# cswaney/NetworkHawkesProcesses.jl

Measured on AMD Instinct MI355X. Metric: log-likelihood evals/sec (N=1024, M=1e6), higher is better.
Workload: dtype f64; 1 GPU; continuous exponential standard Hawkes, N=1024, M=1000000, dt_max=1, windowed_k8 (S-metric, SURVEY 8d); pairs_per_eval=7999107, independent_streams=1

## Files before the change

networkhawkesprocesses.jl_amd/csrc/cont_slices.hip:

```cpp
#include <algorithm>
#include <vector>

#include "nhp_internal.h"
#include "nhp_math.h"
#include "nhp_rng.h"

struct nhp_slices {
    const uint32_t *row;
    const int32_t *item0;
    const uint32_t *lo;
    const uint16_t *hi;
    int32_t nsh;
    uint32_t dmask;
    int32_t dbits;
};

#define NHP_SL_SHARDS 64

#ifdef NHP_STAMP
__device__ unsigned long long g_sl_stamps[8 * 4096];
__device__ unsigned long long g_sl_wave_end[16 * 4096];
#define NHP_SL_STAMP(i) do { if (threadIdx.x == 0 && blockIdx.x < 4096) g_sl_stamps[8 * blockIdx.x + (i)] = __builtin_amdgcn_s_memrealtime(); } while (0)
#define NHP_SL_STAMP_WAVE() do { if ((threadIdx.x & 63) == 0 && blockIdx.x < 4096) g_sl_wave_end[16 * blockIdx.x + (threadIdx.x >> 6)] = __builtin_amdgcn_s_memrealtime(); } while (0)
extern "C" int nhp_debug_stamps_slices(unsigned long long *out, int n)
// ... 147 lines not shown
    for (int k = it.kbeg + threadIdx.x; k < it.kend; k += 256) {
        const nhp_child ch = a.child_w[k];
        const uint32_t slot = (uint32_t)(k - it.kbeg);
        for (int j = ch.idx - 1; j >= ch.first; --j) {
            const nhp_event e = a.ev[j];
            const uint32_t pos = atomicAdd(&cursor[e.node], 1u);
            const int rk = rankof[(size_t)blockIdx.x * N + e.node];
            double q = __builtin_rint((ch.t - e.t) * scale);
            q = q < 1.0 ? 1.0 : (q > qmax ? qmax : q);
            const uint64_t qi = (uint64_t)q;
            const size_t o = ((size_t)row[rk >> 6] + pos) * 64 + (size_t)(rk & 63);
            lo[o] = (uint32_t)qi;
            hi[o] = (uint16_t)((slot << ps.psh) | (uint32_t)(qi >> 32));
        }
    }
    for (int rk = threadIdx.x; rk < ps.spi * 64; rk += 256) {
        const int p = ps.perm[(size_t)blockIdx.x * ps.spi * 64 + rk];
        const uint32_t n = p == 0xFFFF ? 0u : cnt[(size_t)blockIdx.x * N + p];
        const uint32_t r0 = row[rk >> 6], R = row[(rk >> 6) + 1] - r0;
        for (uint32_t i = n; i < R; ++i) {
            const size_t o = ((size_t)r0 + i) * 64 + (size_t)(rk & 63);
            lo[o] = 0;
            hi[o] = (uint16_t)((uint32_t)ps.max_item << ps.psh);
        }
    }
}

__global__ __launch_bounds__(256) void k_ps_sort(int N, nhp_pslices ps, const uint32_t *__restrict__ cnt, uint32_t *__restrict__ lo,
                                                 uint16_t *__restrict__ hi)
{
    const uint32_t *row = ps.row + (size_t)blockIdx.x * ps.spi;
    for (int rk = threadIdx.x; rk < ps.spi * 64; rk += 256) {
        const int p = ps.perm[(size_t)blockIdx.x * ps.spi * 64 + rk];
        if (p == 0xFFFF) continue;
        const int n = (int)cnt[(size_t)blockIdx.x * N + p];
        const size_t o0 = (size_t)row[rk >> 6] * 64 + (size_t)(rk & 63);
        for (int i = 1; i < n; ++i) {
            const uint32_t l = lo[o0 + (size_t)i * 64], h = hi[o0 + (size_t)i * 64];
            const uint64_t key = ((uint64_t)h << 32) | l;
            int j = i - 1;
            while (j >= 0) {
                const uint32_t lj = lo[o0 + (size_t)j * 64], hj = hi[o0 + (size_t)j * 64];
                if ((((uint64_t)hj << 32) | lj) <= key) break;
                lo[o0 + (size_t)(j + 1) * 64] = lj;
                hi[o0 + (size_t)(j + 1) * 64] = (uint16_t)hj;
                --j;
            }
            lo[o0 + (size_t)(j + 1) * 64] = l;
            hi[o0 + (size_t)(j + 1) * 64] = (uint16_t)h;
        }
    }
}

template <int BLOCK, int C, bool FLAT, bool GRAD>
__global__ __launch_bounds__(BLOCK) void k_windowed_slices(nhp_cont_args a, nhp_slices sl, nhp_pslices ps, int mask_integral,
                                                            double *__restrict__ partials, unsigned int *__restrict__ counter,
                                                            double *__restrict__ out, int defer)
{
    constexpr int NW = BLOCK / 64;
    extern __shared__ __align__(16) unsigned char smem[];
    double *red = reinterpret_cast<double *>(smem);
    double2 *col = reinterpret_cast<double2 *>(smem + 320);
    double *etab = reinterpret_cast<double *>(col + a.N + 1);
    double *ginv = etab + 64;
    const int tid = threadIdx.x, lane = tid & 63;
    const double tab_v = nhp_exp2_64[lane];

    const nhp_item it = a.items[blockIdx.x];
    const int c = it.node, N = a.N;
    const int w = __builtin_amdgcn_readfirstlane(tid >> 6);
    const int nchild = it.kend - it.kbeg;
    const int s0 = sl.item0[blockIdx.x], ns = sl.item0[blockIdx.x + 1] - s0;
    NHP_SL_STAMP(0);

    struct chunk { uint32_t lo[C], hi[C]; };
    auto request = [&](chunk &q, const uint32_t *plo, const uint16_t *phi, const uint32_t row0, const int r) {
        const size_t o = ((size_t)row0 + (size_t)r) * 64;
        const uint32_t *pl = plo + o;
        const uint16_t *ph = phi + o;
#pragma unroll
        for (int u = 0; u < C; ++u) {
            q.lo[u] = pl[u * 64 + lane];
            q.hi[u] = ph[u * 64 + lane];
        }
    };
    constexpr int UN = BLOCK >= 512 ? 2 : 4;
    const double unit = __builtin_ldexp(a.dt_max, -sl.dbits);
    int j = w;
    uint32_t row0 = 0;
    int K = 0;
    chunk qa, qb;
    double integ = 0.0;
    for (int p0 = 0; p0 < N; p0 += UN * BLOCK) {
        double w_[UN], th_[UN], a_[UN], cnt_[UN];
#pragma unroll
        for (int u = 0; u < UN; ++u) {
            const int p = p0 + u * BLOCK + tid;
            const size_t k = (size_t)(p < N ? p : 0) + (size_t)c * N;
            w_[u] = a.W[k];
            th_[u] = a.p1[k];
            a_[u] = a.A ? a.A[k] : 1.0;
            cnt_[u] = it.first ? a.cnt[p < N ? p : 0] : 0.0;
        }
        if (p0 == 0) {
            if (j < ns) { row0 = sl.row[s0 + j]; K = (int)(sl.row[s0 + j + 1] - row0); }
            asm volatile("" ::: "memory");
            request(qa, sl.lo, sl.hi, row0, 0);
            asm volatile("" ::: "memory");
        }
#pragma unroll
        for (int u = 0; u < UN; ++u) {
            const int p = p0 + u * BLOCK + tid;
            if (p < N) {
                double wv = w_[u], wint = wv;
                if (a.A) {
                    wv = a_[u] * wv;
                    if (mask_integral) wint = wv;
                }
                col[p] = make_double2(-((th_[u] * unit) * 92.33248261689366), wv * th_[u]);
                integ += cnt_[u] * wint;
            }
        }
    }
    if (tid < 64) etab[tid] = tab_v;
    if (tid == 0) col[N] = make_double2(0.0, 0.0);
    if (GRAD && tid == 0) ginv[ps.max_item] = 0.0;
    if (out && it.first) integ += sl_baseline_integral_col(a, c);
    __syncthreads();
    NHP_SL_STAMP(1);

    const double lam0 = FLAT ? a.lambda0[c] : 0.0;
    const uint32_t dmask = sl.dmask;
    const int nsh = sl.nsh;
    auto delay = [&](const uint32_t lo, const uint32_t h, const uint32_t mask) {
        uint32_t hw;
        asm("v_bfi_b32 %0, %1, %2, %3" : "=v"(hw) : "s"(mask), "v"(h), "v"(0x43300000u));
        return __hiloint2double((int)hw, (int)lo) - 4503599627370496.0;
    };
    auto term = [&](const uint32_t lo, const uint32_t h) {
        const double v = delay(lo, h, dmask);
        const double2 cw = col[h >> nsh];
        return cw.y * nhp_exp_neg_tab_scaled(cw.x * v, etab);
    };
    auto sum = [&](const chunk &q, const int r, const int K, double s) {
        if (r + C <= K) {
            double t[C];
#pragma unroll
            for (int u = 0; u < C; ++u) t[u] = term(q.lo[u], q.hi[u]);
#pragma unroll
            for (int u = 0; u < C; ++u) s += t[u];
        } else {
#pragma unroll
            for (int u = 0; u < C; ++u)
                if (r + u < K) s += term(q.lo[u], q.hi[u]);
        }
        return s;
    };
    double prod = 1.0, gsum = 0.0;
    int pexp = 0;
    int rnd = 0;
    while (j < ns) {
        const int jn = nhp_slice_of(++rnd, w, NW);
        uint32_t row0n = 0;
        int Kn = 0;
        if (jn < ns) { row0n = sl.row[s0 + jn]; Kn = (int)(sl.row[s0 + jn + 1] - row0n); }
        double s = 0.0;
        if (K <= 0) request(qa, sl.lo, sl.hi, row0n, 0);
        for (int r0 = 0; r0 < K; r0 += 2 * C) {
            request(qb, sl.lo, sl.hi, row0, r0 + C);
            asm volatile("" ::: "memory");
            s = sum(qa, r0, K, s);
            const bool more = r0 + 2 * C < K;
            request(qa, sl.lo, sl.hi, more ? row0 : row0n, more ? r0 + 2 * C : 0);
            asm volatile("" ::: "memory");
            s = sum(qb, r0 + C, K, s);
        }
        const int kk = 64 * j + lane;
        if (kk < nchild) {
            const double tk = FLAT ? 0.0 : a.child_w[it.kbeg + kk].t;
            const double lam = (FLAT ? lam0 : sl_baseline(a, c, tk)) + s;
// ... 39 lines not shown
        __syncthreads();
        auto gterm = [&](const uint32_t lo, const uint32_t h, const double xs, double &accH, double &acc1) {
            const double v = delay(lo, h, pmask);
            const double g = ginv[h >> psh];
            const double t = xs * v;
            const double ge = g * nhp_exp_neg_tab_scaled(t, etab);
            accH += ge;
            acc1 = __builtin_fma(ge, __builtin_fma(t, 1.0830424696249145e-02, 1.0), acc1);
        };
        auto gsum_chunk = [&](const chunk &q, const int r, const int K, const double xs, double &accH, double &acc1) {
            if (r + C <= K) {
#pragma unroll
                for (int u = 0; u < C; ++u) gterm(q.lo[u], q.hi[u], xs, accH, acc1);
            } else {
#pragma unroll
                for (int u = 0; u < C; ++u)
                    if (r + u < K) gterm(q.lo[u], q.hi[u], xs, accH, acc1);
            }
        };
        while (jp < ps.spi) {
            const int jn = jp + NW;
            uint32_t row0n = 0;
            int Kn = 0;
            if (jn < ps.spi) { row0n = prow[jn]; Kn = (int)(prow[jn + 1] - row0n); }
            const lanep nxt = lane_params(jn);
            const double xs = -((cur.th * punit) * 92.33248261689366);
            double accH = 0.0, acc1 = 0.0;
            if (Kp <= 0) request(qa, ps.lo, ps.hi, row0n, 0);
            for (int r0 = 0; r0 < Kp; r0 += 2 * C) {
                request(qb, ps.lo, ps.hi, prow0, r0 + C);
                asm volatile("" ::: "memory");
                gsum_chunk(qa, r0, Kp, xs, accH, acc1);
                const bool more = r0 + 2 * C < Kp;
                request(qa, ps.lo, ps.hi, more ? prow0 : row0n, more ? r0 + 2 * C : 0);
                asm volatile("" ::: "memory");
                gsum_chunk(qb, r0 + C, Kp, xs, accH, acc1);
            }
            if (cur.p != 0xFFFF) {
                const size_t k = (size_t)cur.p + (size_t)c * N;
                const double gW = cur.av * (cur.th * accH);
                const double gT = (cur.av * cur.wv) * acc1;
                if (ps.direct) {
                    const double mk = (a.A && mask_integral) ? cur.av : 1.0;
                    ps.grad[L.W + k] = gW - cur.cn * mk;
                    ps.grad[L.p1 + k] = gT;
                } else {
                    if (gW != 0.0) atomicAdd(&ps.grad[L.W + k], gW);
                    if (gT != 0.0) atomicAdd(&ps.grad[L.p1 + k], gT);
                }
            }
            jp = jn; prow0 = row0n; Kp = Kn; cur = nxt;
        }
    }
    double acc = nhp_log(prod) + (double)pexp * 6.93147180559945286e-01;
    if (prod == 0.0) acc = -__builtin_inf();
    double blk = acc, blk_int = integ;
    nhp_block_sum2_n<NW>(blk, blk_int, red);
    if (GRAD && FLAT) {
        const double gs = nhp_block_sum_n<NW>(gsum, red);
        if (tid == 0) {
            if (ps.direct) ps.grad[c] = gs - a.duration;
            else if (gs != 0.0) atomicAdd(&ps.grad[c], gs);
        }
        __syncthreads();
    }
    NHP_SL_STAMP(3);
    if (!out || defer) {
        if (tid == 0) {
            partials[2 * (size_t)blockIdx.x] = blk;
            partials[2 * (size_t)blockIdx.x + 1] = blk_int;
        }
        NHP_SL_STAMP(4);
        return;
    }
    int *flag = reinterpret_cast<int *>(red + 32);
    if (tid == 0) {
        __hip_atomic_store(&partials[2 * (size_t)blockIdx.x], blk, __ATOMIC_RELAXED, __HIP_MEMORY_SCOPE_AGENT);
        __hip_atomic_store(&partials[2 * (size_t)blockIdx.x + 1], blk_int, __ATOMIC_RELAXED, __HIP_MEMORY_SCOPE_AGENT);
        asm volatile("s_waitcnt vmcnt(0)" ::: "memory");
        const unsigned int nb = gridDim.x, sh = blockIdx.x % NHP_SL_SHARDS;
        const unsigned int pop = (nb - sh + NHP_SL_SHARDS - 1) / NHP_SL_SHARDS;
        const unsigned int used = nb < NHP_SL_SHARDS ? nb : NHP_SL_SHARDS;
        int last = 0;
        if (__hip_atomic_fetch_add(&counter[32 * (1 + sh)], 1u, __ATOMIC_RELAXED, __HIP_MEMORY_SCOPE_AGENT) == pop - 1)
            last = __hip_atomic_fetch_add(&counter[0], 1u, __ATOMIC_RELAXED, __HIP_MEMORY_SCOPE_AGENT) == used - 1;
        *flag = last;
    }
    __syncthreads();
    NHP_SL_STAMP(4);
    if (!*flag) return;
    double sl_ = 0.0, si = 0.0;
    for (unsigned int i = tid; i < gridDim.x; i += BLOCK) {
        sl_ += __hip_atomic_load(&partials[2 * (size_t)i], __ATOMIC_RELAXED, __HIP_MEMORY_SCOPE_AGENT);
        si += __hip_atomic_load(&partials[2 * (size_t)i + 1], __ATOMIC_RELAXED, __HIP_MEMORY_SCOPE_AGENT);
    }
    nhp_block_sum2_n<NW>(sl_, si, red);
    if (tid == 0) *out = (0.0 - si) + sl_;
    for (int i = tid; i <= NHP_SL_SHARDS; i += BLOCK)
        __hip_atomic_store(&counter[32 * i], 0u, __ATOMIC_RELAXED, __HIP_MEMORY_SCOPE_AGENT);
}

#define NHP_SETS_MAX 4
struct nhp_sets {
    const double *p1[NHP_SETS_MAX], *W[NHP_SETS_MAX], *A[NHP_SETS_MAX], *lambda0[NHP_SETS_MAX];
    double *out[NHP_SETS_MAX];
};

__device__ __forceinline__ double sl_flat_integral(const double lam0, const double duration)
{
#pragma clang fp contract(off)
    return threadIdx.x == 0 ? lam0 * duration : 0.0;
}

__device__ __forceinline__ double sl_log_of(const double prod, const int pexp)
{
#pragma clang fp contract(off)
    const double e = (double)pexp * 6.93147180559945286e-01;
    return e + nhp_log(prod);
}

template <int BLOCK, int C, int S, bool DEFER = false>
__global__ __launch_bounds__(BLOCK) void k_slices_batch(nhp_cont_args a, nhp_slices sl, nhp_sets st, double *__restrict__ partials,
                                                         unsigned int *__restrict__ counter)
{
    constexpr int NW = BLOCK / 64;
    constexpr bool EARLY = DEFER || (S == 2 && NW <= 8);
    extern __shared__ __align__(16) unsigned char smem[];
    double *red = reinterpret_cast<double *>(smem);
    double2 *col = reinterpret_cast<double2 *>(smem + 320);
    double *etab = reinterpret_cast<double *>(col + (size_t)S * (a.N + 1));
    const int tid = threadIdx.x, lane = tid & 63;
    const double tab_v = nhp_exp2_64[lane];
    const nhp_item it = a.items[blockIdx.x];
    const int c = it.node, N = a.N;
    const int w = __builtin_amdgcn_readfirstlane(tid >> 6);
    const int nchild = it.kend - it.kbeg;
    const int s0 = sl.item0[blockIdx.x], ns = sl.item0[blockIdx.x + 1] - s0;
    NHP_SL_STAMP(0);

    struct chunk { uint32_t lo[C], hi[C]; };
    auto request = [&](chunk &q, const uint32_t row0, const int r) {
        const size_t o = ((size_t)row0 + (size_t)r) * 64;
        const uint32_t *pl = sl.lo + o;
        const uint16_t *ph = sl.hi + o;
#pragma unroll
        for (int u = 0; u < C; ++u) {
            q.lo[u] = pl[u * 64 + lane];
            q.hi[u] = ph[u * 64 + lane];
        }
    };
    constexpr int UN = 2;
    constexpr int G = S >= 2 ? 2 : 1;
    const size_t c0 = (size_t)c * N;
    typedef const __attribute__((address_space(1))) double *gptr;
    gptr Wc[S], Tc[S], Ac[S];
    double lam0[S];
#pragma unroll
    for (int m = 0; m < S; ++m) {
        Wc[m] = (gptr)st.W[m]; Tc[m] = (gptr)st.p1[m]; Ac[m] = (gptr)st.A[m];
        lam0[m] = st.lambda0[m][c];
    }
#pragma unroll
    for (int m = 0; m < S; ++m) asm("" : "+s"(Wc[m]), "+s"(Tc[m]), "+s"(Ac[m]));
    const double unit = __builtin_ldexp(a.dt_max, -sl.dbits);
    int j = w;
    uint32_t row0 = 0;
    int K = 0;
    chunk qa, qb;
    double integ[S];
#pragma unroll
    for (int m = 0; m < S; ++m) integ[m] = 0.0;
    for (int p0 = 0; p0 < N; p0 += UN * BLOCK) {
        double cnt_[UN];
#pragma unroll
        for (int u = 0; u < UN; ++u) {
            const int p = p0 + u * BLOCK + tid;
            cnt_[u] = it.first ? a.cnt[(uint32_t)(p < N ? p : 0)] : 0.0;
        }
#pragma unroll
        for (int g = 0; g < S; g += G) {
            double w_[G][UN], th_[G][UN], a_[G][UN];
#pragma unroll
            for (int mm = 0; mm < G; ++mm) {
                const int m = g + mm;
#pragma unroll
                for (int u = 0; u < UN; ++u) {
                    const int p = p0 + u * BLOCK + tid;
                    const uint32_t k = (uint32_t)(p < N ? p : 0);
                    w_[mm][u] = (Wc[m] + c0)[k];
                    th_[mm][u] = (Tc[m] + c0)[k];
                    a_[mm][u] = Ac[m] ? (Ac[m] + c0)[k] : 1.0;
                }
            }
            if (p0 == 0 && g == 0) {
                if (j < ns) { row0 = sl.row[s0 + j]; K = (int)(sl.row[s0 + j + 1] - row0); }
                asm volatile("" ::: "memory");
                request(qa, row0, 0);
                asm volatile("" ::: "memory");
            }
#pragma unroll
            for (int mm = 0; mm < G; ++mm) {
                const int m = g + mm;
#pragma unroll
                for (int u = 0; u < UN; ++u) {
                    const int p = p0 + u * BLOCK + tid;
                    if (p < N) {
                        double wv = w_[mm][u];
                        if (Ac[m]) wv = a_[mm][u] * wv;
                        col[(size_t)m * (N + 1) + p] = make_double2(-((th_[mm][u] * unit) * 92.33248261689366), wv * th_[mm][u]);
                        if (it.first) integ[m] += cnt_[u] * wv;
                    }
                }
            }
        }
    }
#pragma unroll
    for (int m = 0; m < S; ++m) {
        if (tid == 0) col[(size_t)m * (N + 1) + N] = make_double2(0.0, 0.0);
        if (DEFER) {
            if (it.first) integ[m] += sl_flat_integral(lam0[m], a.duration);
        } else if (it.first && tid == 0) integ[m] += lam0[m] * a.duration;
        if (EARLY) {
            const double wsum = nhp_wave_sum(integ[m]);
            if (lane == 0) red[16 + m * NW + w] = wsum;
        }
    }
    if (tid < 64) etab[tid] = tab_v;
    __syncthreads();
    NHP_SL_STAMP(1);

    const uint32_t dmask = sl.dmask;
    const int nsh = sl.nsh;
    const uint32_t plane = (uint32_t)(N + 1) * 16u;
    auto terms = [&](const uint32_t lo, const uint32_t h, double (&acc)[S]) {
        uint32_t hw;
        asm("v_bfi_b32 %0, %1, %2, %3" : "=v"(hw) : "s"(dmask), "v"(h), "v"(0x43300000u));
        const double v = __hiloint2double((int)hw, (int)lo) - 4503599627370496.0;
        const unsigned char *base = reinterpret_cast<const unsigned char *>(col) + ((h >> nsh) << 4);
#pragma unroll
        for (int m = 0; m < S; ++m) {
            const double2 cw = *reinterpret_cast<const double2 *>(base + m * plane);
            acc[m] = __builtin_fma(cw.y, nhp_exp_neg_tab_scaled(cw.x * v, etab), acc[m]);
        }
    };
    auto sum = [&](const chunk &q, const int r, const int K, double (&acc)[S]) {
        if (r + C <= K) {
#pragma unroll
            for (int u = 0; u < C; ++u) terms(q.lo[u], q.hi[u], acc);
        } else {
#pragma unroll
            for (int u = 0; u < C; ++u)
                if (r + u < K) terms(q.lo[u], q.hi[u], acc);
        }
    };
    double prod[S];
    int pexp[S];
#pragma unroll
    for (int m = 0; m < S; ++m) { prod[m] = 1.0; pexp[m] = 0; }
    int rnd = 0;
    while (j < ns) {
        const int jn = nhp_slice_of(++rnd, w, NW);
        uint32_t row0n = 0;
        int Kn = 0;
        if (jn < ns) { row0n = sl.row[s0 + jn]; Kn = (int)(sl.row[s0 + jn + 1] - row0n); }
        double acc[S];
#pragma unroll
        for (int m = 0; m < S; ++m) acc[m] = 0.0;
        if (K <= 0) request(qa, row0n, 0);
        for (int r0 = 0; r0 < K; r0 += 2 * C) {
            request(qb, row0, r0 + C);
            asm volatile("" ::: "memory");
            sum(qa, r0, K, acc);
            const bool more = r0 + 2 * C < K;
            request(qa, more ? row0 : row0n, more ? r0 + 2 * C : 0);
            asm volatile("" ::: "memory");
            sum(qb, r0 + C, K, acc);
        }
        const int kk = 64 * j + lane;
        if (kk < nchild) {
#pragma unroll
            for (int m = 0; m < S; ++m) {
                const double lam = lam0[m] + acc[m];
                prod[m] *= lam < 0.0 ? __builtin_nan("") : __builtin_amdgcn_frexp_mant(lam);
                pexp[m] += __builtin_amdgcn_frexp_exp(lam);
            }
        }
#pragma unroll
        for (int m = 0; m < S; ++m) {
            pexp[m] += __builtin_amdgcn_frexp_exp(prod[m]);
            prod[m] = __builtin_amdgcn_frexp_mant(prod[m]);
        }
        j = jn; row0 = row0n; K = Kn;
    }
    NHP_SL_STAMP_WAVE();
    NHP_SL_STAMP(2);
    if (DEFER) {
        double ws[S];
#pragma unroll
        for (int m = 0; m < S; ++m) {
            double blk = sl_log_of(prod[m], pexp[m]);
            if (prod[m] == 0.0) blk = -__builtin_inf();
            ws[m] = nhp_wave_sum(blk);
        }
        __syncthreads();
        if (lane == 0) {
#pragma unroll
            for (int m = 0; m < S; ++m) red[m * NW + w] = ws[m];
        }
        __syncthreads();
        NHP_SL_STAMP(3);
        if (tid == 0) {
#pragma unroll
            for (int m = 0; m < S; ++m) {
                double sx = 0.0, sy = 0.0;
                for (int q = 0; q < NW; ++q) { sx += red[m * NW + q]; sy += red[16 + m * NW + q]; }
                st.out[m][2 * (size_t)blockIdx.x] = sx;
                st.out[m][2 * (size_t)blockIdx.x + 1] = sy;
            }
        }
        NHP_SL_STAMP(4);
        return;
    }
    int *flag = reinterpret_cast<int *>(red + 32);
#pragma unroll
    for (int m = 0; m < S; ++m) {
        double blk = nhp_log(prod[m]) + (double)pexp[m] * 6.93147180559945286e-01;
        if (prod[m] == 0.0) blk = -__builtin_inf();
        double blk_int = EARLY ? 0.0 : integ[m];
        nhp_block_sum2_n<NW>(blk, blk_int, red);
        if (EARLY && tid == 0)
            for (int q = 0; q < NW; ++q) blk_int += red[16 + m * NW + q];
        if (tid == 0) {
            __hip_atomic_store(&partials[(2 * (size_t)blockIdx.x) * S + 2 * m], blk, __ATOMIC_RELAXED, __HIP_MEMORY_SCOPE_AGENT);
            __hip_atomic_store(&partials[(2 * (size_t)blockIdx.x) * S + 2 * m + 1], blk_int, __ATOMIC_RELAXED, __HIP_MEMORY_SCOPE_AGENT);
        }
        __syncthreads();
    }
    NHP_SL_STAMP(3);
    if (tid == 0) {
        asm volatile("s_waitcnt vmcnt(0)" ::: "memory");
        const unsigned int nb = gridDim.x, sh = blockIdx.x % NHP_SL_SHARDS;
        const unsigned int pop = (nb - sh + NHP_SL_SHARDS - 1) / NHP_SL_SHARDS;
        const unsigned int used = nb < NHP_SL_SHARDS ? nb : NHP_SL_SHARDS;
        int last = 0;
        if (__hip_atomic_fetch_add(&counter[32 * (1 + sh)], 1u, __ATOMIC_RELAXED, __HIP_MEMORY_SCOPE_AGENT) == pop - 1)
            last = __hip_atomic_fetch_add(&counter[0], 1u, __ATOMIC_RELAXED, __HIP_MEMORY_SCOPE_AGENT) == used - 1;
        *flag = last;
    }
    __syncthreads();
    NHP_SL_STAMP(4);
    if (!*flag) return;
#pragma unroll
    for (int m = 0; m < S; ++m) {
        double sl_ = 0.0, si = 0.0;
        for (unsigned int i = tid; i < gridDim.x; i += BLOCK) {
            sl_ += __hip_atomic_load(&partials[(2 * (size_t)i) * S + 2 * m], __ATOMIC_RELAXED, __HIP_MEMORY_SCOPE_AGENT);
            si += __hip_atomic_load(&partials[(2 * (size_t)i) * S + 2 * m + 1], __ATOMIC_RELAXED, __HIP_MEMORY_SCOPE_AGENT);
        }
        nhp_block_sum2_n<NW>(sl_, si, red);
        if (tid == 0) *st.out[m] = (0.0 - si) + sl_;
        __syncthreads();
    }
    for (int i = tid; i <= NHP_SL_SHARDS; i += BLOCK)
        __hip_atomic_store(&counter[32 * i], 0u, __ATOMIC_RELAXED, __HIP_MEMORY_SCOPE_AGENT);
}

__global__ __launch_bounds__(256) void k_slices_build_lq(nhp_cont_args a, nhp_slices sl, double *__restrict__ L, double *__restrict__ Q)
{
#pragma clang fp contract(off)
    const nhp_item it = a.items[blockIdx.x];
    const int lane = threadIdx.x & 63, w = threadIdx.x >> 6;
    const int nchild = it.kend - it.kbeg;
    const int s0 = sl.item0[blockIdx.x], ns = sl.item0[blockIdx.x + 1] - s0;
    for (int j = w; j < ns; j += 4) {
        const uint32_t row0 = sl.row[s0 + j];
        const int K = (int)(sl.row[s0 + j + 1] - row0);
        const int kk = 64 * j + lane;
        nhp_child ch;
        ch.t = 0.0; ch.first = 0; ch.idx = 0;
        if (kk < nchild) ch = a.child_w[it.kbeg + kk];
        const int len = ch.idx - ch.first;
        for (int r = 0; r < K; ++r) {
            double2 d = make_double2(0.0, 0.0);
            if (r < len) d = nhp_logitnormal_data(a.inv_dtmax, ch.t - a.ev[ch.idx - 1 - r].t);
            const size_t o = ((size_t)row0 + (size_t)r) * 64 + (size_t)lane;
            L[o] = d.x;
            Q[o] = d.y;
        }
    }
}

__global__ __launch_bounds__(256) void k_slices_build_d(nhp_cont_args a, nhp_slices sl, double *__restrict__ D)
// ... 332 lines not shown
    if (hipMalloc((void **)&d_cnt, 4 * (size_t)ni * N) != hipSuccess || hipMalloc((void **)&d_rows, 4 * (size_t)ni * spi) != hipSuccess ||
        hipMalloc((void **)&d_rankof, 2 * (size_t)ni * N) != hipSuccess ||
        hipMalloc((void **)&ds->d_ps_perm, 2 * (size_t)ni * spi * 64) != hipSuccess ||
        hipMalloc((void **)&ds->d_ps_row, 4 * ((size_t)ni * spi + 1)) != hipSuccess)
        return fail(NHP_ENOMEM, "out of device memory");
    const size_t lds = 4 * (size_t)N;
    if (lds > 64 * 1024) {
        (void)hipFuncSetAttribute((const void *)k_ps_count, hipFuncAttributeMaxDynamicSharedMemorySize, (int)lds);
        (void)hipFuncSetAttribute((const void *)k_ps_rank, hipFuncAttributeMaxDynamicSharedMemorySize, (int)lds);
        (void)hipFuncSetAttribute((const void *)k_ps_fill, hipFuncAttributeMaxDynamicSharedMemorySize, (int)lds);
    }
    hipLaunchKernelGGL(k_ps_count, dim3((unsigned)ni), dim3(256), lds, ctx->main(), a, d_cnt);
    hipLaunchKernelGGL(k_ps_rank, dim3((unsigned)ni), dim3(256), lds, ctx->main(), N, spi, d_cnt, ds->d_ps_perm, d_rankof, d_rows);
    if (hipGetLastError() != hipSuccess) return fail(NHP_EHIP, "launch failed");
    std::vector<uint32_t> rows((size_t)ni * spi), off((size_t)ni * spi + 1);
    if (hipMemcpyAsync(rows.data(), d_rows, 4 * rows.size(), hipMemcpyDeviceToHost, ctx->main()) != hipSuccess ||
        hipStreamSynchronize(ctx->main()) != hipSuccess) return fail(NHP_EHIP, "copy failed");
    uint64_t run = 0;
    for (size_t q = 0; q < rows.size(); ++q) { off[q] = (uint32_t)run; run += rows[q]; }
    off[rows.size()] = (uint32_t)run;
    if (run >= ((uint64_t)1 << 25)) return fail(NHP_ENOTIMPL, "too many rows");
    ds->ps_rows = (int64_t)run; ds->ps_spi = spi; ds->ps_sb = sb;
    const size_t n = ((size_t)run + 16) * 64;
    if (hipMalloc((void **)&ds->d_ps_lo, 4 * n) != hipSuccess || hipMalloc((void **)&ds->d_ps_hi, 2 * n) != hipSuccess)
        return fail(NHP_ENOMEM, "out of device memory");
    if (hipMemcpyAsync(ds->d_ps_row, off.data(), 4 * off.size(), hipMemcpyHostToDevice, ctx->main()) != hipSuccess ||
        hipMemsetAsync(ds->d_ps_lo + (size_t)run * 64, 0, 4 * 16 * 64, ctx->main()) != hipSuccess ||
        hipMemsetAsync(ds->d_ps_hi + (size_t)run * 64, 0, 2 * 16 * 64, ctx->main()) != hipSuccess)
        return fail(NHP_EHIP, "copy failed");
    const nhp_pslices ps = pslices_view(ds);
    hipLaunchKernelGGL(k_ps_fill, dim3((unsigned)ni), dim3(256), lds, ctx->main(), a, ps, d_cnt, d_rankof, ds->d_ps_lo, ds->d_ps_hi);
    hipLaunchKernelGGL(k_ps_sort, dim3((unsigned)ni), dim3(256), 0, ctx->main(), N, ps, d_cnt, ds->d_ps_lo, ds->d_ps_hi);
    if (hipGetLastError() != hipSuccess || hipStreamSynchronize(ctx->main()) != hipSuccess) return fail(NHP_EHIP, "fill failed");
    (void)hipFree(d_cnt); (void)hipFree(d_rows); (void)hipFree(d_rankof);
    return NHP_OK;
}

static void slices_cfg(const nhp_cont_dataset *ds, int *B, int *C)
{
    const int per_item = (ds->max_item + 63) / 64;
    const double mean_rows = ds->n_slices > 0 ? (double)ds->sl_rows / (double)ds->n_slices : 0.0;
    *B = per_item >= 12 ? 512 : per_item >= 6 ? 256 : per_item >= 3 ? 128 : 64;
    *C = mean_rows >= 48.0 ? 8 : mean_rows >= 16.0 ? 4 : 2;
    if (const char *cfg = getenv("NHP_SLICES_CFG")) sscanf(cfg, "%d,%d", B, C);
}

static nhp_status launch_slices(nhp_ctx *ctx, const nhp_cont_dataset *ds, const nhp_cont_model *m, int mask_integral, double *d_out,
                                double *d_grad, bool direct, bool *launched, int32_t defer_slot = -1, bool *deferred = nullptr)
{
    *launched = false;
    if (deferred) *deferred = false;
    if (!ds->d_sl_row || ds->n_items <= 0 || m->impulse_kind != NHP_IMPULSE_EXPONENTIAL) return NHP_OK;
    if (nhp_slices_off(d_grad ? "NHP_GRAD_SLICES" : nullptr)) return NHP_OK;
    const size_t lds = 320 + 16 * ((size_t)ds->N + 1) + 512 + (d_grad ? 8 * ((size_t)ds->max_item + 1) : 0);
    if (lds > 160 * 1024) return NHP_OK;
    NHP_HIP(ctx, hipSetDevice(ctx->device));
    NHP_TRY(nhp_ctx_reserve_partials(ctx, 2 * (size_t)ds->n_items));
    nhp_cont_args a = nhp_make_args(ds, m);
    NHP_TRY(ensure_slices(ctx, ds, a));
    const nhp_slices sl = slices_view(ds);
    nhp_pslices ps{};
    if (d_grad) {
        NHP_TRY(ensure_parent_slices(ctx, ds, a));
        ps = pslices_view(ds);
        ps.grad = d_grad;
        ps.direct = direct ? 1 : 0;
    }
    int B, C;
    slices_cfg(ds, &B, &C);
    dim3 grid((unsigned)ds->n_items);
    bool ok = false;
    const bool flat = m->baseline_kind == NHP_BASELINE_HOMOGENEOUS;
    const bool known = (B == 64 || B == 128 || B == 256 || B == 512) && (C == 2 || C == 4 || C == 8);
    const int defer = defer_slot >= 0 && !d_grad && d_out && known ? 1 : 0;
    double *partials = ctx->d_partials;
    if (defer) {
        NHP_TRY(nhp_ctx_reserve_slot_partials(ctx, defer_slot, 2 * (size_t)ds->n_items));
        partials = ctx->d_slot_partials[defer_slot];
    }
#define NHP_SLAUNCH(b, cc, f, g)                                                                                      \
    do {                                                                                                              \
        if (lds > 64 * 1024)                                                                                          \
            (void)hipFuncSetAttribute((const void *)k_windowed_slices<b, cc, f, g>, hipFuncAttributeMaxDynamicSharedMemorySize, (int)lds); \
        hipLaunchKernelGGL((k_windowed_slices<b, cc, f, g>), grid, dim3(b), lds, ctx->lane(), a, sl, ps, mask_integral, partials, \
                           ctx->d_counter, d_out, defer);                                                             \
    } while (0)
#define NHP_SCASE(b, cc)                                                                                              \
    if (!ok && B == b && C == cc) {                                                                                   \
        ok = true;                                                                                                    \
        if (d_grad) { if (flat) NHP_SLAUNCH(b, cc, true, true); else NHP_SLAUNCH(b, cc, false, true); }               \
        else { if (flat) NHP_SLAUNCH(b, cc, true, false); else NHP_SLAUNCH(b, cc, false, false); }                    \
    }
#define NHP_SROW(b) NHP_SCASE(b, 2) NHP_SCASE(b, 4) NHP_SCASE(b, 8)
    NHP_SROW(64) NHP_SROW(128) NHP_SROW(256) NHP_SROW(512) NHP_SROW(1024)
    if (!ok) { B = 256; C = 4; NHP_SCASE(256, 4) }
#undef NHP_SLAUNCH
#undef NHP_SROW
#undef NHP_SCASE
    NHP_HIP(ctx, hipGetLastError());
    if (defer) {
        ctx->pend.mark(defer_slot, ds->n_items, B);
        if (deferred) *deferred = true;
    }
    *launched = true;
    return NHP_OK;
}

// ... 72 lines not shown
    return ds->all_sole && !nhp_is_column_shard(ds) && m->baseline_kind == NHP_BASELINE_HOMOGENEOUS;
}

extern "C" int64_t nhp_debug_parent_slices(const nhp_cont_dataset *ds, uint32_t *lo, uint16_t *hi, int64_t cap)
{
    if (!ds || !ds->d_ps_lo) return -1;
    const int64_t n = ds->ps_rows * 64;
    if (lo && hi && cap >= n) {
        if (hipMemcpy(lo, ds->d_ps_lo, 4 * (size_t)n, hipMemcpyDeviceToHost) != hipSuccess) return -2;
        if (hipMemcpy(hi, ds->d_ps_hi, 2 * (size_t)n, hipMemcpyDeviceToHost) != hipSuccess) return -2;
    }
    return n;
}

template <int S>
static nhp_status launch_sets(nhp_ctx *ctx, const nhp_cont_dataset *ds, const nhp_cont_model *const *ms, int32_t slot0, size_t lds)
{
    NHP_TRY(nhp_ctx_reserve_partials(ctx, 2 * (size_t)ds->n_items * S));
    nhp_cont_args a = nhp_make_args(ds, ms[0]);
    NHP_TRY(ensure_slices(ctx, ds, a));
    const nhp_slices sl = slices_view(ds);
    nhp_sets st;
    for (int k = 0; k < NHP_SETS_MAX; ++k) {
        const nhp_cont_model *m = ms[k < S ? k : 0];
        st.p1[k] = m->d_p1; st.W[k] = m->d_W; st.A[k] = m->has_A ? m->d_A : nullptr; st.lambda0[k] = m->d_lambda0;
        st.out[k] = ctx->d_results + slot0 + (k < S ? k : 0);
    }
    const double mean_rows = ds->n_slices > 0 ? (double)ds->sl_rows / (double)ds->n_slices : 0.0;
    dim3 grid((unsigned)ds->n_items);
    int B = (ds->max_item + 63) / 64 >= 6 ? 512 : 256, C = mean_rows >= 16.0 ? 4 : 2;
    if (const char *cfg = getenv("NHP_SETS_CFG")) sscanf(cfg, "%d,%d", &B, &C);
#define NHP_BL(b, cc)                                                                                                  \
    do {                                                                                                               \
        if (lds > 64 * 1024)                                                                                           \
            (void)hipFuncSetAttribute((const void *)k_slices_batch<b, cc, S>, hipFuncAttributeMaxDynamicSharedMemorySize, (int)lds); \
        hipLaunchKernelGGL((k_slices_batch<b, cc, S>), grid, dim3(b), lds, ctx->lane(), a, sl, st, ctx->d_partials, ctx->d_counter); \
    } while (0)
    if (B == 256 && C == 2) NHP_BL(256, 2); else if (B == 256) NHP_BL(256, 4);
    else if (B == 1024 && C == 2) NHP_BL(1024, 2); else if (B == 1024) NHP_BL(1024, 4);
    else if (C == 2) NHP_BL(512, 2); else NHP_BL(512, 4);
#undef NHP_BL
    NHP_HIP(ctx, hipGetLastError());
    return NHP_OK;
}

nhp_status nhp_launch_slices_batch(nhp_ctx *ctx, const nhp_cont_dataset *ds, const nhp_cont_model *const *ms, int S, int32_t slot0,
                                   bool *launched)
{
    *launched = false;
    if (!ds->d_sl_row || ds->n_items <= 0 || (S != 2 && S != 4)) return NHP_OK;
    if (nhp_slices_off("NHP_BATCH_SLICES")) return NHP_OK;
    for (int k = 0; k < S; ++k)
        if (!ms[k] || ms[k]->impulse_kind != NHP_IMPULSE_EXPONENTIAL || ms[k]->baseline_kind != NHP_BASELINE_HOMOGENEOUS) return NHP_OK;
    const size_t lds = 320 + 16 * ((size_t)ds->N + 1) * (size_t)S + 512;
    if (lds > 160 * 1024) return NHP_OK;
    NHP_HIP(ctx, hipSetDevice(ctx->device));
    if (S == 4) NHP_TRY(launch_sets<4>(ctx, ds, ms, slot0, lds)); else NHP_TRY(launch_sets<2>(ctx, ds, ms, slot0, lds));
    *launched = true;
    return NHP_OK;
}

bool nhp_slices_pair_eligible(const nhp_cont_dataset *ds, const nhp_cont_model *m)
{
    if (!ds || !m || !ds->d_sl_row || ds->n_items <= 0) return false;
    if (m->impulse_kind != NHP_IMPULSE_EXPONENTIAL || m->baseline_kind != NHP_BASELINE_HOMOGENEOUS) return false;
    if (!ds->all_sole || nhp_is_column_shard(ds) || nhp_slices_off(nullptr)) return false;
    if (const char *pl = getenv("NHP_PLIST")) if (atoi(pl) == 0) return false;
    if (4 * (320 + 32 * ((size_t)ds->N + 1) + 512) > 160 * 1024) return false;
    int B, C;
    slices_cfg(ds, &B, &C);
    return (B == 64 || B == 128 || B == 256 || B == 512) && (C == 2 || C == 4 || C == 8);
}

nhp_status nhp_launch_slices_pair(nhp_ctx *ctx, const nhp_cont_dataset *ds, const nhp_cont_model *const *ms, const int32_t *slot)
{
    const size_t lds = 320 + 32 * ((size_t)ds->N + 1) + 512;
    NHP_HIP(ctx, hipSetDevice(ctx->device));
    for (int k = 0; k < 2; ++k) NHP_TRY(nhp_ctx_reserve_slot_partials(ctx, slot[k], 2 * (size_t)ds->n_items));
    nhp_cont_args a = nhp_make_args(ds, ms[0]);
    NHP_TRY(ensure_slices(ctx, ds, a));
    const nhp_slices sl = slices_view(ds);
    nhp_sets st;
    for (int k = 0; k < NHP_SETS_MAX; ++k) {
        const nhp_cont_model *m = ms[k & 1];
        st.p1[k] = m->d_p1; st.W[k] = m->d_W; st.A[k] = m->has_A ? m->d_A : nullptr; st.lambda0[k] = m->d_lambda0;
        st.out[k] = ctx->d_slot_partials[slot[k & 1]];
    }
    int B, C;
    slices_cfg(ds, &B, &C);
    dim3 grid((unsigned)ds->n_items);
    bool ok = false;
#define NHP_PCASE(b, cc)                                                                                              \
    if (!ok && B == b && C == cc) {                                                                                   \
        ok = true;                                                                                                    \
        if (lds > 64 * 1024)                                                                                          \
            (void)hipFuncSetAttribute((const void *)k_slices_batch<b, cc, 2, true>, hipFuncAttributeMaxDynamicSharedMemorySize, (int)lds); \
        hipLaunchKernelGGL((k_slices_batch<b, cc, 2, true>), grid, dim3(b), lds, ctx->lane(), a, sl, st, (double *)nullptr,  \
                           (unsigned int *)nullptr);                                                                  \
    }
#define NHP_PROW(b) NHP_PCASE(b, 2) NHP_PCASE(b, 4) NHP_PCASE(b, 8)
    NHP_PROW(64) NHP_PROW(128) NHP_PROW(256) NHP_PROW(512)
#undef NHP_PROW
#undef NHP_PCASE
    if (!ok) { nhp_set_error(ctx, "paired enqueue: no kernel for %d threads, %d rows", B, C); return NHP_EINVAL; }
    NHP_HIP(ctx, hipGetLastError());
    for (int k = 0; k < 2; ++k) ctx->pend.mark(slot[k], ds->n_items, B);
    return NHP_OK;
}

static nhp_status ensure_lq_planes(nhp_ctx *ctx, nhp_cont_dataset *ds, const nhp_cont_args &a, const nhp_slices &sl, bool *ok)
{
    *ok = true;
    if (ds->d_sl_L) return NHP_OK;
    const size_t n = ((size_t)ds->sl_rows + 16) * 64;
    if (hipMalloc((void **)&ds->d_sl_L, 8 * n) != hipSuccess || hipMalloc((void **)&ds->d_sl_Q, 8 * n) != hipSuccess) {
        (void)hipGetLastError();
        (void)hipFree(ds->d_sl_L); (void)hipFree(ds->d_sl_Q);
        ds->d_sl_L = nullptr; ds->d_sl_Q = nullptr;
        *ok = false;
        return NHP_OK;
    }
    NHP_HIP(ctx, hipMemsetAsync(ds->d_sl_L + (size_t)ds->sl_rows * 64, 0, 8 * 16 * 64, ctx->main()));
    NHP_HIP(ctx, hipMemsetAsync(ds->d_sl_Q + (size_t)ds->sl_rows * 64, 0, 8 * 16 * 64, ctx->main()));
    hipLaunchKernelGGL(k_slices_build_lq, dim3((unsigned)ds->n_items), dim3(256), 0, ctx->main(), a, sl, ds->d_sl_L, ds->d_sl_Q);
    NHP_HIP(ctx, hipGetLastError());
    return NHP_OK;
}

nhp_status nhp_launch_sampler_slices(nhp_ctx *ctx, const nhp_cont_dataset *cds, const nhp_cont_model *m, const double *d_u, uint64_t seed,
// ... 51 lines not shown
```

Before: 101,500 log-likelihood evals/sec.

## Reduce per-wave products before log and park integral partials early in LDS

At the end of the slices kernels, the code no longer takes a log per lane followed by a block sum. Each wave now multiplies its lane products with DPP and readlane, folds the exponents separately, and takes a single log per wave from frexp mantissa and exponent. The integral partials are also reduced to quarter-wave values and parked in LDS before the main loop, so the exit needs one barrier instead of repeated block reductions. This trades per-lane transcendental work and synchronisation for extra LDS and a risk of changed rounding or overflow handling in the product.

```diff
diff --git a/networkhawkesprocesses.jl_amd/csrc/cont_slices.hip b/networkhawkesprocesses.jl_amd/csrc/cont_slices.hip
--- a/networkhawkesprocesses.jl_amd/csrc/cont_slices.hip
+++ b/networkhawkesprocesses.jl_amd/csrc/cont_slices.hip
@@ -223,6 +223,89 @@
     }
 }
 
+__host__ __device__ constexpr size_t sl_exit_bytes(const int S, const int NW) { return ((size_t)S * NW * (17 * 8 + 8 + 4) + 15) / 16 * 16; }
+
+__device__ __forceinline__ double sl_dpp_mul(const double v, const int sel)
+{
+#pragma clang fp contract(off)
+    const int lo = __double2loint(v), hi = __double2hiint(v);
+    int plo, phi;
+    switch (sel) {
+    case 0: plo = __builtin_amdgcn_mov_dpp(lo, 0xB1, 0xF, 0xF, true); phi = __builtin_amdgcn_mov_dpp(hi, 0xB1, 0xF, 0xF, true); break;
+    case 1: plo = __builtin_amdgcn_mov_dpp(lo, 0x4E, 0xF, 0xF, true); phi = __builtin_amdgcn_mov_dpp(hi, 0x4E, 0xF, 0xF, true); break;
+    case 2: plo = __builtin_amdgcn_mov_dpp(lo, 0x141, 0xF, 0xF, true); phi = __builtin_amdgcn_mov_dpp(hi, 0x141, 0xF, 0xF, true); break;
+    default: plo = __builtin_amdgcn_mov_dpp(lo, 0x140, 0xF, 0xF, true); phi = __builtin_amdgcn_mov_dpp(hi, 0x140, 0xF, 0xF, true); break;
+    }
+    return v * __hiloint2double(phi, plo);
+}
+
+template <int NW>
+__device__ __forceinline__ void sl_exit_park(double v, double *__restrict__ park, const int m, const int w, const int lane)
+{
+#pragma clang fp contract(off)
+    v = nhp_dpp_add(v, 0);
+    v = nhp_dpp_add(v, 1);
+    if ((lane & 3) == 0) park[(m * NW + w) * 17 + (lane >> 2)] = v;
+}
+
+template <int NW, int S>
+__device__ __forceinline__ void sl_exit_sums(const double (&prod)[S], const int (&pexp)[S], double *__restrict__ park, double (&sx)[S], double (&sy)[S])
+{
+#pragma clang fp contract(off)
+    constexpr int Q = S * NW;
+    static_assert(Q <= 64, "one lane of the first wave per (model, wave)");
+    double *mant = park + Q * 17;
+    int *wexp = reinterpret_cast<int *>(mant + Q);
+    const int tid = threadIdx.x, lane = tid & 63;
+    const int w = __builtin_amdgcn_readfirstlane(tid >> 6);
+#pragma unroll
+    for (int m = 0; m < S; ++m) {
+        double p = prod[m];
+        p = sl_dpp_mul(p, 0);
+        p = sl_dpp_mul(p, 1);
+        p = sl_dpp_mul(p, 2);
+        p = sl_dpp_mul(p, 3);
+        const int lo = __double2loint(p), hi = __double2hiint(p);
+        double r = __hiloint2double(__builtin_amdgcn_readlane(hi, 0), __builtin_amdgcn_readlane(lo, 0));
+        r *= __hiloint2double(__builtin_amdgcn_readlane(hi, 16), __builtin_amdgcn_readlane(lo, 16));
+        r *= __hiloint2double(__builtin_amdgcn_readlane(hi, 32), __builtin_amdgcn_readlane(lo, 32));
+        r *= __hiloint2double(__builtin_amdgcn_readlane(hi, 48), __builtin_amdgcn_readlane(lo, 48));
+        int e = pexp[m];
+        e += __builtin_amdgcn_mov_dpp(e, 0xB1, 0xF, 0xF, true);
+        e += __builtin_amdgcn_mov_dpp(e, 0x4E, 0xF, 0xF, true);
+        e += __builtin_amdgcn_mov_dpp(e, 0x141, 0xF, 0xF, true);
+        e += __builtin_amdgcn_mov_dpp(e, 0x140, 0xF, 0xF, true);
+        const int es = __builtin_amdgcn_readlane(e, 0) + __builtin_amdgcn_readlane(e, 16) + __builtin_amdgcn_readlane(e, 32) +
+                       __builtin_amdgcn_readlane(e, 48) + __builtin_amdgcn_frexp_exp(r);
+        if (lane == 0) {
+            mant[m * NW + w] = __builtin_amdgcn_frexp_mant(r);
+            wexp[m * NW + w] = es;
+        }
+    }
+    __syncthreads();
+    if (w != 0) return;
+    if (lane < Q) {
+        const double lg = nhp_log(mant[lane]) + (double)wexp[lane] * 6.93147180559945286e-01;
+        double *pk = park + lane * 17;
+        double si = 0.0;
+#pragma unroll
+        for (int i = 0; i < 16; ++i) si += pk[i];
+        mant[lane] = lg;
+        pk[0] = si;
+    }
+    __builtin_amdgcn_fence(__ATOMIC_RELEASE, "wavefront");
+    __builtin_amdgcn_wave_barrier();
+    __builtin_amdgcn_fence(__ATOMIC_ACQUIRE, "wavefront");
+    if (tid == 0) {
+#pragma unroll
+        for (int m = 0; m < S; ++m) {
+            double x = 0.0, y = 0.0;
+            for (int q = 0; q < NW; ++q) { x += mant[m * NW + q]; y += park[(m * NW + q) * 17]; }
+            sx[m] = x; sy[m] = y;
+        }
+    }
+}
+
 template <int BLOCK, int C, bool FLAT, bool GRAD>
 __global__ __launch_bounds__(BLOCK) void k_windowed_slices(nhp_cont_args a, nhp_slices sl, nhp_pslices ps, int mask_integral,
                                                             double *__restrict__ partials, unsigned int *__restrict__ counter,
@@ -234,6 +317,7 @@
     double2 *col = reinterpret_cast<double2 *>(smem + 320);
     double *etab = reinterpret_cast<double *>(col + a.N + 1);
     double *ginv = etab + 64;
+    double *park = etab + 64;
     const int tid = threadIdx.x, lane = tid & 63;
     const double tab_v = nhp_exp2_64[lane];
 
@@ -297,6 +381,7 @@
     if (tid == 0) col[N] = make_double2(0.0, 0.0);
     if (GRAD && tid == 0) ginv[ps.max_item] = 0.0;
     if (out && it.first) integ += sl_baseline_integral_col(a, c);
+    if (!GRAD) sl_exit_park<NW>(integ, park, 0, w, lane);
     __syncthreads();
     NHP_SL_STAMP(1);
 
@@ -442,10 +527,19 @@
             jp = jn; prow0 = row0n; Kp = Kn; cur = nxt;
         }
     }
-    double acc = nhp_log(prod) + (double)pexp * 6.93147180559945286e-01;
-    if (prod == 0.0) acc = -__builtin_inf();
-    double blk = acc, blk_int = integ;
-    nhp_block_sum2_n<NW>(blk, blk_int, red);
+    double blk = 0.0, blk_int = 0.0;
+    if constexpr (GRAD) {
+        double acc = nhp_log(prod) + (double)pexp * 6.93147180559945286e-01;
+        if (prod == 0.0) acc = -__builtin_inf();
+        blk = acc; blk_int = integ;
+        nhp_block_sum2_n<NW>(blk, blk_int, red);
+    } else {
+        const double p1[1] = {prod};
+        const int e1[1] = {pexp};
+        double sx[1] = {0.0}, sy[1] = {0.0};
+        sl_exit_sums<NW, 1>(p1, e1, park, sx, sy);
+        blk = sx[0]; blk_int = sy[0];
+    }
     if (GRAD && FLAT) {
         const double gs = nhp_block_sum_n<NW>(gsum, red);
         if (tid == 0) {
@@ -502,23 +596,16 @@
     return threadIdx.x == 0 ? lam0 * duration : 0.0;
 }
 
-__device__ __forceinline__ double sl_log_of(const double prod, const int pexp)
-{
-#pragma clang fp contract(off)
-    const double e = (double)pexp * 6.93147180559945286e-01;
-    return e + nhp_log(prod);
-}
-
 template <int BLOCK, int C, int S, bool DEFER = false>
 __global__ __launch_bounds__(BLOCK) void k_slices_batch(nhp_cont_args a, nhp_slices sl, nhp_sets st, double *__restrict__ partials,
                                                          unsigned int *__restrict__ counter)
 {
     constexpr int NW = BLOCK / 64;
-    constexpr bool EARLY = DEFER || (S == 2 && NW <= 8);
     extern __shared__ __align__(16) unsigned char smem[];
     double *red = reinterpret_cast<double *>(smem);
     double2 *col = reinterpret_cast<double2 *>(smem + 320);
     double *etab = reinterpret_cast<double *>(col + (size_t)S * (a.N + 1));
+    double *park = etab + 64;
     const int tid = threadIdx.x, lane = tid & 63;
     const double tab_v = nhp_exp2_64[lane];
     const nhp_item it = a.items[blockIdx.x];
@@ -607,13 +694,8 @@
 #pragma unroll
     for (int m = 0; m < S; ++m) {
         if (tid == 0) col[(size_t)m * (N + 1) + N] = make_double2(0.0, 0.0);
-        if (DEFER) {
-            if (it.first) integ[m] += sl_flat_integral(lam0[m], a.duration);
-        } else if (it.first && tid == 0) integ[m] += lam0[m] * a.duration;
-        if (EARLY) {
-            const double wsum = nhp_wave_sum(integ[m]);
-            if (lane == 0) red[16 + m * NW + w] = wsum;
-        }
+        if (it.first) integ[m] += sl_flat_integral(lam0[m], a.duration);
+        sl_exit_park<NW>(integ[m], park, m, w, lane);
     }
     if (tid < 64) etab[tid] = tab_v;
     __syncthreads();
@@ -684,50 +766,29 @@
     }
     NHP_SL_STAMP_WAVE();
     NHP_SL_STAMP(2);
+    double sx[S], sy[S];
+#pragma unroll
+    for (int m = 0; m < S; ++m) { sx[m] = 0.0; sy[m] = 0.0; }
+    sl_exit_sums<NW, S>(prod, pexp, park, sx, sy);
+    NHP_SL_STAMP(3);
     if (DEFER) {
-        double ws[S];
-#pragma unroll
-        for (int m = 0; m < S; ++m) {
-            double blk = sl_log_of(prod[m], pexp[m]);
-            if (prod[m] == 0.0) blk = -__builtin_inf();
-            ws[m] = nhp_wave_sum(blk);
-        }
-        __syncthreads();
-        if (lane == 0) {
-#pragma unroll
-            for (int m = 0; m < S; ++m) red[m * NW + w] = ws[m];
-        }
-        __syncthreads();
-        NHP_SL_STAMP(3);
         if (tid == 0) {
 #pragma unroll
             for (int m = 0; m < S; ++m) {
-                double sx = 0.0, sy = 0.0;
-                for (int q = 0; q < NW; ++q) { sx += red[m * NW + q]; sy += red[16 + m * NW + q]; }
-                st.out[m][2 * (size_t)blockIdx.x] = sx;
-                st.out[m][2 * (size_t)blockIdx.x + 1] = sy;
+                st.out[m][2 * (size_t)blockIdx.x] = sx[m];
+                st.out[m][2 * (size_t)blockIdx.x + 1] = sy[m];
             }
         }
         NHP_SL_STAMP(4);
         return;
     }
     int *flag = reinterpret_cast<int *>(red + 32);
-#pragma unroll
-    for (int m = 0; m < S; ++m) {
-        double blk = nhp_log(prod[m]) + (double)pexp[m] * 6.93147180559945286e-01;
-        if (prod[m] == 0.0) blk = -__builtin_inf();
-        double blk_int = EARLY ? 0.0 : integ[m];
-        nhp_block_sum2_n<NW>(blk, blk_int, red);
-        if (EARLY && tid == 0)
-            for (int q = 0; q < NW; ++q) blk_int += red[16 + m * NW + q];
-        if (tid == 0) {
-            __hip_atomic_store(&partials[(2 * (size_t)blockIdx.x) * S + 2 * m], blk, __ATOMIC_RELAXED, __HIP_MEMORY_SCOPE_AGENT);
-            __hip_atomic_store(&partials[(2 * (size_t)blockIdx.x) * S + 2 * m + 1], blk_int, __ATOMIC_RELAXED, __HIP_MEMORY_SCOPE_AGENT);
-        }
-        __syncthreads();
-    }
-    NHP_SL_STAMP(3);
     if (tid == 0) {
+#pragma unroll
+        for (int m = 0; m < S; ++m) {
+            __hip_atomic_store(&partials[(2 * (size_t)blockIdx.x) * S + 2 * m], sx[m], __ATOMIC_RELAXED, __HIP_MEMORY_SCOPE_AGENT);
+            __hip_atomic_store(&partials[(2 * (size_t)blockIdx.x) * S + 2 * m + 1], sy[m], __ATOMIC_RELAXED, __HIP_MEMORY_SCOPE_AGENT);
+        }
         asm volatile("s_waitcnt vmcnt(0)" ::: "memory");
         const unsigned int nb = gridDim.x, sh = blockIdx.x % NHP_SL_SHARDS;
         const unsigned int pop = (nb - sh + NHP_SL_SHARDS - 1) / NHP_SL_SHARDS;
@@ -1166,7 +1227,7 @@
     if (deferred) *deferred = false;
     if (!ds->d_sl_row || ds->n_items <= 0 || m->impulse_kind != NHP_IMPULSE_EXPONENTIAL) return NHP_OK;
     if (nhp_slices_off(d_grad ? "NHP_GRAD_SLICES" : nullptr)) return NHP_OK;
-    const size_t lds = 320 + 16 * ((size_t)ds->N + 1) + 512 + (d_grad ? 8 * ((size_t)ds->max_item + 1) : 0);
+    const size_t lds = 320 + 16 * ((size_t)ds->N + 1) + 512 + (d_grad ? 8 * ((size_t)ds->max_item + 1) : sl_exit_bytes(1, 16));
     if (lds > 160 * 1024) return NHP_OK;
     NHP_HIP(ctx, hipSetDevice(ctx->device));
     NHP_TRY(nhp_ctx_reserve_partials(ctx, 2 * (size_t)ds->n_items));
@@ -1345,7 +1406,7 @@
     if (nhp_slices_off("NHP_BATCH_SLICES")) return NHP_OK;
     for (int k = 0; k < S; ++k)
         if (!ms[k] || ms[k]->impulse_kind != NHP_IMPULSE_EXPONENTIAL || ms[k]->baseline_kind != NHP_BASELINE_HOMOGENEOUS) return NHP_OK;
-    const size_t lds = 320 + 16 * ((size_t)ds->N + 1) * (size_t)S + 512;
+    const size_t lds = 320 + 16 * ((size_t)ds->N + 1) * (size_t)S + 512 + sl_exit_bytes(S, 16);
     if (lds > 160 * 1024) return NHP_OK;
     NHP_HIP(ctx, hipSetDevice(ctx->device));
     if (S == 4) NHP_TRY(launch_sets<4>(ctx, ds, ms, slot0, lds)); else NHP_TRY(launch_sets<2>(ctx, ds, ms, slot0, lds));
@@ -1359,7 +1420,7 @@
     if (m->impulse_kind != NHP_IMPULSE_EXPONENTIAL || m->baseline_kind != NHP_BASELINE_HOMOGENEOUS) return false;
     if (!ds->all_sole || nhp_is_column_shard(ds) || nhp_slices_off(nullptr)) return false;
     if (const char *pl = getenv("NHP_PLIST")) if (atoi(pl) == 0) return false;
-    if (4 * (320 + 32 * ((size_t)ds->N + 1) + 512) > 160 * 1024) return false;
+    if (4 * (320 + 32 * ((size_t)ds->N + 1) + 512 + sl_exit_bytes(2, 8)) > 160 * 1024) return false;
     int B, C;
     slices_cfg(ds, &B, &C);
     return (B == 64 || B == 128 || B == 256 || B == 512) && (C == 2 || C == 4 || C == 8);
@@ -1367,7 +1428,7 @@
 
 nhp_status nhp_launch_slices_pair(nhp_ctx *ctx, const nhp_cont_dataset *ds, const nhp_cont_model *const *ms, const int32_t *slot)
 {
-    const size_t lds = 320 + 32 * ((size_t)ds->N + 1) + 512;
+    const size_t lds = 320 + 32 * ((size_t)ds->N + 1) + 512 + sl_exit_bytes(2, 8);
     NHP_HIP(ctx, hipSetDevice(ctx->device));
     for (int k = 0; k < 2; ++k) NHP_TRY(nhp_ctx_reserve_slot_partials(ctx, slot[k], 2 * (size_t)ds->n_items));
     nhp_cont_args a = nhp_make_args(ds, ms[0]);
```

After: 110,200 log-likelihood evals/sec (median of 6 runs). +8.6%, better.
